# yeyupiaoling/VoiceprintRecognition-PaddlePaddle

Hardware: NVIDIA H100
Metric: utterances/sec ECAPA-TDNN Fbank80 3s embed extract (higher is better)
Workload: dtype bf16x3 (split-bf16 operands, fp32 accumulate; fp32-grade)

## Files before the change

voiceprintrecognition-paddlepaddle_b200/csrc/gemm_epilogue.cuh:

```cuda
#pragma once
#include "common.h"
#include "ptx.cuh"

namespace ppv {

constexpr int GEMM_MMA_THREADS = 256;
constexpr int GEMM_THREADS = 128 + GEMM_MMA_THREADS;

__device__ __forceinline__ float epilogue_math1(const Epilogue& ep, int N, int col, int64_t grp, int64_t sgrp, float x) {
    if (ep.bias) x += __ldg(ep.bias + col);
    if (ep.rowgrp_bias) x += __ldg(ep.rowgrp_bias + grp * N + col);
    if (ep.seg_scale) x *= __ldg(ep.seg_scale + sgrp * N + col);
    if (ep.relu) {
        x = fmaxf(x, 0.f);
        if (ep.relu_max > 0.f) x = fminf(x, ep.relu_max);
    }
    if (ep.silu_) x = x / (1.f + expf(-x));
    if (ep.bn_scale) x = fmaf(x, __ldg(ep.bn_scale + col), __ldg(ep.bn_shift + col));
    if (ep.tanh_) x = tanhf(x);
    if (ep.sigmoid_) x = 1.f / (1.f + expf(-x));
    return x;
}

struct EpiRow {
    bool valid = false;
    int64_t out_row = 0, mirror_a = -1, mirror_b = -1, grp = 0, sgrp = 0;
    int64_t zero_row = -1;
};
__device__ __forceinline__ EpiRow epilogue_row(const Epilogue& ep, int64_t row, int64_t out_row_shift) {
    EpiRow r;
    r.valid = row >= 0;
    const int64_t row_in = row;
    if (row < 0) row = 0;
    r.out_row = row + out_row_shift;
    if (ep.img_Wp > 0) {
        const int64_t img = int64_t(ep.img_Hp) * ep.img_Wp;
        r.grp = row / img;
        const int rem = int(row - r.grp * img);
        const int h = rem / ep.img_Wp - 1, w = rem % ep.img_Wp - 1;
        r.valid = r.valid && h >= 0 && h < ep.img_H && w >= 0 && w < ep.img_W;
        const int sw = ep.img_stride_w ? ep.img_stride_w : ep.img_stride;
        r.valid = r.valid && (h % ep.img_stride) == 0 && (w % sw) == 0;
        r.out_row = (r.grp * ep.out_Hp + h / ep.img_stride + 1) * ep.out_Wp + w / sw + 1;
    } else if (ep.Tp > 0) {
        r.grp = row / ep.Tp;
        const int t = int(row - r.grp * ep.Tp) - ep.P;
        r.valid = r.valid && t >= 0 && t < ep.T;
        if (ep.seg_scale && r.valid) r.sgrp = r.grp * ep.nseg + t / ep.seg_len;
        if (ep.halo && r.valid) {
            if (t >= 1 && t <= ep.P) r.mirror_a = row - 2 * t;
            const int u = ep.T - 1 - t;
            if (u >= 1 && u <= ep.P) r.mirror_b = row + 2 * u;
        }
    }
    const bool same_grid = ep.img_Wp == 0 || (ep.img_stride == 1 && ep.img_stride_w <= 1 && ep.out_Hp == ep.img_Hp && ep.out_Wp == ep.img_Wp);
    if (!r.valid && row_in >= 0 && ep.zero_invalid && ep.out_mode == OUT_PLANES && !ep.halo && same_grid) r.zero_row = row_in + out_row_shift;
    return r;
}

__device__ __forceinline__ void epilogue_pair(const Epilogue& ep, int N, int col, const EpiRow& r, float a, float b) {
    if (col >= N) return;
    if (!r.valid) {
        if (r.zero_row >= 0) {
            __nv_bfloat16* ph = static_cast<__nv_bfloat16*>(ep.out) + r.zero_row * ep.out_ld + ep.out_col0 + col;
            *reinterpret_cast<uint32_t*>(ph) = 0u;
            *reinterpret_cast<uint32_t*>(ph + ep.out_plane_stride) = 0u;
        }
        return;
    }
    const bool two = col + 1 < N;
    a = epilogue_math1(ep, N, col, r.grp, r.sgrp, a);
    if (two) b = epilogue_math1(ep, N, col + 1, r.grp, r.sgrp, b);
    if (ep.out_mode == OUT_F32) {
        float* dst = static_cast<float*>(ep.out) + r.out_row * ep.out_ld + ep.out_col0 + col;
        if (two && ep.f32_vec_ok) {
            *reinterpret_cast<float2*>(dst) = make_float2(a, b);
        } else {
            dst[0] = a;
            if (two) dst[1] = b;
        }
        return;
    }
    uint32_t h, l;
    split_pack_bf16x2(a, b, h, l);
    __nv_bfloat16* obase = static_cast<__nv_bfloat16*>(ep.out) + ep.out_col0 + col;
    auto store_row = [&](int64_t row) {
        uint32_t* ph = reinterpret_cast<uint32_t*>(obase + row * ep.out_ld);
        ph[0] = h;
        *reinterpret_cast<uint32_t*>(reinterpret_cast<__nv_bfloat16*>(ph) + ep.out_plane_stride) = l;
    };
    store_row(r.out_row);
    if (r.mirror_a >= 0) store_row(r.mirror_a);
    if (r.mirror_b >= 0) store_row(r.mirror_b);
}

template <int BN, typename RowOf>
__device__ __forceinline__ void epilogue_frag(const Epilogue& ep, int N, int n0, float (&acc)[BN / 2], RowOf&& row_of, int t,
                                              int64_t out_row_shift = 0) {
    if (ep.debug_nostore) return;
    const int w = t >> 5, l = t & 31;
    const int r0 = 16 * w + (l >> 2);
    const EpiRow ra = epilogue_row(ep, row_of(r0), out_row_shift);
    const EpiRow rb = epilogue_row(ep, row_of(r0 + 8), out_row_shift);
    constexpr int EPI_GROUPS = BN / 8 < 4 ? BN / 8 : 4;
#pragma unroll 1
    for (int c = 0; c < BN / 8; c += EPI_GROUPS) {
#pragma unroll
        for (int i = 0; i < EPI_GROUPS; ++i) {
            const int col = n0 + 8 * (c + i) + 2 * (l & 3);
            epilogue_pair(ep, N, col, ra, acc[4 * i + 0], acc[4 * i + 1]);
            epilogue_pair(ep, N, col, rb, acc[4 * i + 2], acc[4 * i + 3]);
        }
#pragma unroll
        for (int j = 0; j + 4 * EPI_GROUPS < BN / 2; ++j) acc[j] = acc[j + 4 * EPI_GROUPS];
    }
}

template <int BN, typename RowOf>
__device__ __forceinline__ void epilogue_frag_lean(const Epilogue& ep, int N, int n0, float (&acc)[BN / 2], RowOf&& row_of, int t) {
    static_assert(BN % 32 == 0, "lean epilogue: whole 32-column trips");
    const int w = t >> 5, l = t & 31, q = l & 3;
    const int r0 = 16 * w + (l >> 2);
    const EpiRow ra = epilogue_row(ep, row_of(r0), 0);
    const EpiRow rb = epilogue_row(ep, row_of(r0 + 8), 0);
    const int cq = n0 + 8 * q;
    __nv_bfloat16* const obase = static_cast<__nv_bfloat16*>(ep.out) + ep.out_col0 + cq;
    __nv_bfloat16* const pa = obase + ra.out_row * ep.out_ld;
    __nv_bfloat16* const pb = obase + rb.out_row * ep.out_ld;
    const int64_t lo_off = ep.out_plane_stride;
    const float* const ga = ep.rowgrp_bias ? ep.rowgrp_bias + ra.grp * N + cq : nullptr;
    const float* const gb = ep.rowgrp_bias ? ep.rowgrp_bias + rb.grp * N + cq : nullptr;
    const bool q2 = (q & 2) != 0, q1 = (q & 1) != 0;
#pragma unroll 1
    for (int c = 0; c < BN / 8; c += 4) {
        float a[8], b[8];
#pragma unroll
        for (int i = 0; i < 4; ++i) a[2 * i] = acc[4 * i], a[2 * i + 1] = acc[4 * i + 1], b[2 * i] = acc[4 * i + 2], b[2 * i + 1] = acc[4 * i + 3];
#pragma unroll
        for (int j = 0; j + 16 < BN / 2; ++j) acc[j] = acc[j + 16];
#pragma unroll
        for (int e = 0; e < 4; ++e) {
            const float sa = q2 ? a[e] : a[e + 4], sb = q2 ? b[e] : b[e + 4];
            const float ra_ = __shfl_xor_sync(0xffffffffu, sa, 2), rb_ = __shfl_xor_sync(0xffffffffu, sb, 2);
            if (q2) a[e] = ra_, b[e] = rb_;
            else a[e + 4] = ra_, b[e + 4] = rb_;
        }
#pragma unroll
        for (int e = 0; e < 8; e += 4) {
#pragma unroll
            for (int f = 0; f < 2; ++f) {
                const float sa = q1 ? a[e + f] : a[e + 2 + f], sb = q1 ? b[e + f] : b[e + 2 + f];
                const float ra_ = __shfl_xor_sync(0xffffffffu, sa, 1), rb_ = __shfl_xor_sync(0xffffffffu, sb, 1);
                if (q1) a[e + f] = ra_, b[e + f] = rb_;
                else a[e + 2 + f] = ra_, b[e + 2 + f] = rb_;
            }
        }
        const int j0 = 8 * c;
        if (n0 + j0 >= N) continue;
#pragma unroll
        for (int k = 0; k < 8; ++k) {
            const int col = cq + j0 + k;
            if (ep.bias) {
                const float bb = __ldg(ep.bias + col);
                a[k] += bb, b[k] += bb;
            }
            if (ga) a[k] += __ldg(ga + j0 + k), b[k] += __ldg(gb + j0 + k);
            if (ep.relu) a[k] = fmaxf(a[k], 0.f), b[k] = fmaxf(b[k], 0.f);
            if (ep.bn_scale) {
                const float sc = __ldg(ep.bn_scale + col), sh = __ldg(ep.bn_shift + col);
                a[k] = fmaf(a[k], sc, sh), b[k] = fmaf(b[k], sc, sh);
            }
            if (ep.tanh_) a[k] = tanhf(a[k]), b[k] = tanhf(b[k]);
        }
        uint4 ha, la, hb, lb;
        split_pack_bf16x2(a[0], a[1], ha.x, la.x), split_pack_bf16x2(a[2], a[3], ha.y, la.y);
        split_pack_bf16x2(a[4], a[5], ha.z, la.z), split_pack_bf16x2(a[6], a[7], ha.w, la.w);
        split_pack_bf16x2(b[0], b[1], hb.x, lb.x), split_pack_bf16x2(b[2], b[3], hb.y, lb.y);
        split_pack_bf16x2(b[4], b[5], hb.z, lb.z), split_pack_bf16x2(b[6], b[7], hb.w, lb.w);
        if (ra.valid) {
            *reinterpret_cast<uint4*>(pa + j0) = ha;
            *reinterpret_cast<uint4*>(pa + j0 + lo_off) = la;
        }
        if (rb.valid) {
            *reinterpret_cast<uint4*>(pb + j0) = hb;
            *reinterpret_cast<uint4*>(pb + j0 + lo_off) = lb;
        }
    }
}

template <int BN, typename RowOf>
__device__ __forceinline__ void gemm_epilogue(const Epilogue& ep, int N, int n0, float (&acc)[BN / 2], RowOf&& row_of, int t,
                                              int64_t out_row_shift) {
    if (ep.lean) epilogue_frag_lean<BN>(ep, N, n0, acc, row_of, t);
    else epilogue_frag<BN>(ep, N, n0, acc, row_of, t, out_row_shift);
}

}
```

voiceprintrecognition-paddlepaddle_b200/csrc/res2chain.cu:

```cuda
#include <stdio.h>
#include <stdlib.h>
#include <string.h>

#include "common.h"
#include "gemm_epilogue.cuh"
#include "ptx.cuh"

namespace ppv {

constexpr int RC_PAD = 4;
constexpr int RC_BOX_ROWS = 200;
constexpr int RC_ROWS = 2 * RC_BOX_ROWS;
constexpr int RC_A_PLANE = RC_ROWS * 128;
constexpr int RC_W_TILE = 64 * 128;
constexpr int RC_MAX_TILES = 3;
constexpr int RC_MAX_TP = RC_MAX_TILES * GEMM_BM;
constexpr int RC_S_PLANE = GEMM_BM * 128;
constexpr int RC_MMA_THREADS = 128 * RC_MAX_TILES;
constexpr int RC_THREADS = 128 + RC_MMA_THREADS;

template <int NSPLIT>
struct RCCfg {
    static constexpr int NP = (NSPLIT == 3) ? 2 : 1;
    static constexpr int A_BYTES = NP * RC_A_PLANE;
    static constexpr int W_SLOT = 3 * NP * RC_W_TILE;
    static constexpr int S_BYTES = NP * RC_S_PLANE;
    static constexpr int SMEM_BYTES = 1024 + A_BYTES + W_SLOT + 2 * S_BYTES + 256;
};

__device__ __forceinline__ void rp_st_global(bool pred, uint32_t* p, uint32_t v) {
    asm volatile("{\n\t.reg .pred p;\n\tsetp.ne.b32 p, %2, 0;\n\t@p st.global.u32 [%0], %1;\n\t}" ::"l"(p), "r"(v), "r"(uint32_t(pred)) : "memory");
}
__device__ __forceinline__ void rp_st_shared(bool pred, uint32_t a, uint32_t v) {
    asm volatile("{\n\t.reg .pred p;\n\tsetp.ne.b32 p, %2, 0;\n\t@p st.shared.u32 [%0], %1;\n\t}" ::"r"(a), "r"(v), "r"(uint32_t(pred)) : "memory");
}

__device__ __forceinline__ uint32_t rc_ld_shared(uint32_t a) {
    uint32_t v;
    asm volatile("ld.shared.u32 %0, [%1];" : "=r"(v) : "r"(a) : "memory");
    return v;
}

#define RC_STAMP(role, conv, ev)                                                                   \
    do {                                                                                          \
        if (cp.trace && blockIdx.x == 0 && b == 0) cp.trace[((role) * 8 + (conv)) * 8 + (ev)] = clock64(); \
    } while (0)

template <int NSPLIT>
__global__ void __launch_bounds__(RC_THREADS, 1) res2chain_kernel(const __grid_constant__ Res2ChainParams cp) {
    using Cfg = RCCfg<NSPLIT>;
    constexpr int NP = Cfg::NP, BN = 64;
    extern __shared__ uint8_t smem_raw[];
    const uint32_t smem_base = (smem_u32(smem_raw) + 1023u) & ~1023u;
    uint8_t* smem_gen = smem_raw + (smem_base - smem_u32(smem_raw));
    const uint32_t a_base = smem_base;
    const uint32_t w_base = a_base + Cfg::A_BYTES;
    const uint32_t s_base = w_base + Cfg::W_SLOT;
    const uint32_t bar_base = s_base + 2 * Cfg::S_BYTES;
    const uint32_t x_full = bar_base, x_free = bar_base + 24, w_full = bar_base + 32, w_empty = bar_base + 40;
    auto s_full = [&](int i) { return bar_base + 48u + 8u * i; };
    auto s_empty = [&](int i) { return bar_base + 64u + 8u * i; };
    auto y_ready = [&](int i) { return bar_base + 80u + 8u * i; };

    const int warp = threadIdx.x >> 5, lane = threadIdx.x & 31;
    if (warp == 0 && lane == 0) {
        prefetch_tmap(&cp.mapX);
        prefetch_tmap(&cp.mapXt);
        prefetch_tmap(&cp.mapY);
        prefetch_tmap(&cp.mapYtail);
        for (int j = 0; j < cp.nconv; ++j) prefetch_tmap(&cp.mapW[j]);
    }
    if (warp == 1 && lane == 0) {
        mbar_init(x_full, 1);
        mbar_init(x_free, 1);
        mbar_init(w_full, 1);
        mbar_init(w_empty, 1);
        for (int i = 0; i < 2; ++i) {
            mbar_init(s_full(i), 1);
            mbar_init(s_empty(i), 1);
            mbar_init(y_ready(i), 128);
        }
        fence_mbar_init();
    }
    __syncthreads();
    griddep_launch_dependents();
    const int nconv = cp.nconv, ntiles = cp.ntiles;

    if (warp == 0) {
        if (lane == 0) {
            griddep_wait();
            int g = 0, u = 0;
            uint32_t sn = 0;
            for (int b = blockIdx.x; b < cp.B; b += gridDim.x, ++u) {
                if (u > 0) mbar_wait(x_free, uint32_t(u - 1) & 1u);
                mbar_arrive_expect_tx(x_full, NP * 2 * RC_BOX_ROWS * 128);
                for (int pl = 0; pl < NP; ++pl)
                    for (int h = 0; h < 2; ++h)
                        tma_load_3d(a_base + pl * RC_A_PLANE + h * RC_BOX_ROWS * 128, &cp.mapX, x_full, cp.width ,
                                    b * cp.Tp - RC_PAD + h * RC_BOX_ROWS, pl);
                for (int j = 0; j < nconv; ++j, ++g) {
                    if (g > 0) mbar_wait(w_empty, uint32_t(g - 1) & 1u);
                    RC_STAMP(0, j, 0);
                    mbar_arrive_expect_tx(w_full, 3 * NP * RC_W_TILE);
                    for (int tap = 0; tap < 3; ++tap)
                        for (int pl = 0; pl < NP; ++pl) tma_load_3d(w_base + (tap * NP + pl) * RC_W_TILE, &cp.mapW[j], w_full, tap * 64, 0, pl);
                    for (int t = 0; t < ntiles; ++t, ++sn) {
                        const int i = sn & 1;
                        if (sn >= 2) mbar_wait(s_empty(i), ((sn >> 1) - 1) & 1u);
                        if (j + 1 < nconv) {
                            mbar_arrive_expect_tx(s_full(i), NP * RC_S_PLANE);
                            for (int pl = 0; pl < NP; ++pl)
                                tma_load_3d(s_base + i * Cfg::S_BYTES + pl * RC_S_PLANE, &cp.mapXt, s_full(i), (j + 2) * cp.width,
                                            b * cp.Tp + t * GEMM_BM, pl);
                        } else {
                            mbar_arrive(s_full(i));
                        }
                    }
                }
            }
        }
    } else if (warp == 3) {
        if (lane == 0) {
            uint32_t sn = 0;
            for (int b = blockIdx.x; b < cp.B; b += gridDim.x) {
                for (int j = 0; j < nconv; ++j) {
                    for (int t = 0; t < ntiles; ++t, ++sn) {
                        const int i = sn & 1;
                        mbar_wait(y_ready(i), (sn >> 1) & 1u);
                        const CUtensorMap* my = (t == ntiles - 1) ? &cp.mapYtail : &cp.mapY;
                        for (int pl = 0; pl < NP; ++pl)
                            tma_store_3d(my, s_base + i * Cfg::S_BYTES + pl * RC_S_PLANE, (j + 1) * cp.width, b * cp.Tp + t * GEMM_BM, pl);
                        bulk_commit_group();
                        bulk_wait_read0();
                        mbar_arrive(s_empty(i));
                    }
                }
            }
            bulk_wait_all();
        }
    } else if (warp >= 4) {
        const int tw = (warp - 4) >> 2, tid = threadIdx.x & 127, w = tid >> 5, l = tid & 31;
        const int e = threadIdx.x - 128;
        const bool has_tile = tw < ntiles;
        griddep_wait();
        uint8_t* const a_gen = smem_gen;
        float acc0[BN / 2], acc1[BN / 2];
#pragma unroll
        for (int i = 0; i < BN / 2; ++i) acc0[i] = acc1[i] = 0.f;
        uint32_t g = 0, ucount = 0;
        for (int b = blockIdx.x; b < cp.B; b += gridDim.x, ++ucount) {
            {
                mbar_wait(x_full, ucount & 1u);
                if (e < 2 * cp.P * 8 * NP) {
                    const int pl = e / (2 * cp.P * 8), r = (e / 8) % (2 * cp.P), c = e % 8;
                    const int k = (r % cp.P) + 1;
                    const int dst = (r < cp.P ? cp.P - k : cp.P + cp.T - 1 + k) + RC_PAD, src = (r < cp.P ? cp.P + k : cp.P + cp.T - 1 - k) + RC_PAD;
                    const uint4 val = *reinterpret_cast<const uint4*>(a_gen + pl * RC_A_PLANE + src * 128 + ((c ^ (src & 7)) << 4));
                    *reinterpret_cast<uint4*>(a_gen + pl * RC_A_PLANE + dst * 128 + ((c ^ (dst & 7)) << 4)) = val;
                }
                fence_proxy_async_smem();
                named_bar_sync(1, RC_MMA_THREADS);
            }
            for (int j = 0; j < nconv; ++j, ++g) {
                mbar_wait(w_full, g & 1u);
                if (tid == 0 && tw == 0) RC_STAMP(1, j, 1);
                if (has_tile) {
                    wgmma_fence_acc(acc0);
                    wgmma_fence_acc(acc1);
                    wgmma_fence();
                    auto issue = [&](float (&acc)[BN / 2], int mb) {
#pragma unroll
                        for (int tap = 0; tap < 3; ++tap) {
                            const uint32_t roff = uint32_t(tw * GEMM_BM + mb * 64 + RC_PAD + (tap - 1) * cp.dil);
                            const uint64_t a_hi = make_sw128_kmajor_desc(a_base + roff * 128u);
                            const uint64_t b_hi = make_sw128_kmajor_desc(w_base + (tap * NP) * RC_W_TILE);
#pragma unroll
                            for (int k = 0; k < 4; ++k) wgmma_bf16<BN>(acc, a_hi + 2 * k, b_hi + 2 * k, (tap > 0 || k > 0) ? 1u : 0u);
                            if (NSPLIT == 3) {
                                const uint64_t a_lo = make_sw128_kmajor_desc(a_base + RC_A_PLANE + roff * 128u);
                                const uint64_t b_lo = make_sw128_kmajor_desc(w_base + (tap * NP + 1) * RC_W_TILE);
#pragma unroll
                                for (int k = 0; k < 4; ++k) wgmma_bf16<BN>(acc, a_lo + 2 * k, b_hi + 2 * k, 1u);
#pragma unroll
                                for (int k = 0; k < 4; ++k) wgmma_bf16<BN>(acc, a_hi + 2 * k, b_lo + 2 * k, 1u);
                            }
                        }
                    };
                    issue(acc0, 0);
                    issue(acc1, 1);
                    wgmma_commit();
                    wgmma_wait<0>();
                    wgmma_fence_acc(acc0);
                    wgmma_fence_acc(acc1);
                }
                named_bar_sync(1, RC_MMA_THREADS);
                if (e == 0) {
                    RC_STAMP(1, j, 2);
                    mbar_arrive(w_empty);
                    if (j == nconv - 1) mbar_arrive(x_free);
                }
                const float* bias = cp.bias[j];
                const float* bsc = cp.bn_scale[j];
                const float* bsh = cp.bn_shift[j];
                const bool has_next = j + 1 < nconv;
                const uint32_t sn = g * uint32_t(ntiles) + uint32_t(tw);
                const int i = sn & 1;
                auto epilogue = [&](const float (&acc)[BN / 2], int mb) {
#pragma unroll 1
                    for (int h = 0; h < 2; ++h) {
                        const int rloc = mb * 64 + 16 * w + (l >> 2) + 8 * h;
                        const int p = tw * GEMM_BM + rloc;
                        const int tt = p - cp.P, uu = cp.T - 1 - tt;
                        const bool next = has_next && tt >= 0 && tt < cp.T;
                        const int m0 = p + RC_PAD;
                        const int m1 = (tt >= 1 && tt <= cp.P) ? cp.P - tt + RC_PAD : -1;
                        const int m2 = (uu >= 1 && uu <= cp.P) ? cp.P + cp.T - 1 + uu + RC_PAD : -1;
                        const uint32_t srow = s_base + i * Cfg::S_BYTES + rloc * 128 + 4 * (l & 3);
#pragma unroll
                        for (int q = 0; q < BN / 8; ++q) {
                            const int col = 8 * q + 2 * (l & 3);
                            const uint32_t so = srow + ((q ^ (rloc & 7)) << 4);
                            const float2 b2 = __ldg(reinterpret_cast<const float2*>(bias + col));
                            const float2 s2 = __ldg(reinterpret_cast<const float2*>(bsc + col));
                            const float2 h2 = __ldg(reinterpret_cast<const float2*>(bsh + col));
                            const float a0 = h ? acc[4 * q + 2] : acc[4 * q], a1 = h ? acc[4 * q + 3] : acc[4 * q + 1];
                            const float x0 = fmaf(fmaxf(a0 + b2.x, 0.f), s2.x, h2.x);
                            const float x1 = fmaf(fmaxf(a1 + b2.y, 0.f), s2.y, h2.y);
                            uint32_t nh = 0, nl = 0;
                            if (has_next) {
                                nh = rc_ld_shared(so);
                                if (NP == 2) nl = rc_ld_shared(so + RC_S_PLANE);
                            }
                            uint32_t yh, yl;
                            split_pack_bf16x2(x0, x1, yh, yl);
                            rp_st_shared(true, so, yh);
                            if (NP == 2) rp_st_shared(true, so + RC_S_PLANE, yl);
                            const float2 hf = unpack_bf16x2(nh), lf = unpack_bf16x2(nl);
                            uint32_t oh, ol;
                            split_pack_bf16x2(x0 + (hf.x + lf.x), x1 + (hf.y + lf.y), oh, ol);
                            auto put = [&](bool pred, int row) {
                                const uint32_t d = a_base + row * 128 + ((q ^ (row & 7)) << 4) + 4 * (l & 3);
                                rp_st_shared(pred, d, oh);
                                if (NP == 2) rp_st_shared(pred, d + RC_A_PLANE, ol);
                            };
                            put(next, m0);
                            put(next && m1 >= 0, m1);
                            put(next && m2 >= 0, m2);
                        }
                    }
                };
#pragma unroll 1
                for (int round = 0; round < 2; ++round) {
                    if (has_tile && (tw == 2) == (round == 1)) {
                        mbar_wait(s_full(i), (sn >> 1) & 1u);
                        epilogue(acc0, 0);
                        epilogue(acc1, 1);
                        fence_proxy_async_smem();
                        mbar_arrive(y_ready(i));
                    }
                    if (ntiles > 2 && round == 0) named_bar_sync(2, RC_MMA_THREADS);
                }
                if (tid == 0 && tw == 0) RC_STAMP(2, j, 5);
                if (has_next) {
                    fence_proxy_async_smem();
                    named_bar_sync(1, RC_MMA_THREADS);
                }
            }
        }
    }
}

constexpr int RP_BLOCKS = 5;
constexpr int RP_MAX_TP = RP_BLOCKS * 64;
constexpr int RP_BOX_ROWS = 168;
constexpr int RP_A_PLANE = 2 * RP_BOX_ROWS * 128;
constexpr int RP_THREADS = 128 * RP_BLOCKS;
constexpr int RP_VEC_FLOATS = 3 * RES2CHAIN_MAX * 64;

template <int NSPLIT>
struct RPCfg {
    static constexpr int NP = (NSPLIT == 3) ? 2 : 1;
    static constexpr int U_BYTES = NP * RP_A_PLANE;
    static constexpr int W_SLOT = 3 * NP * RC_W_TILE;
    static constexpr int SMEM_BYTES = 1024 + 2 * U_BYTES + W_SLOT + RP_VEC_FLOATS * 4 + 64;
};
static_assert(RPCfg<3>::SMEM_BYTES <= 232448, "paired res2chain exceeds the H100 shared-memory opt-in");

#define RP_STAMP(role, conv, ev)                                                                                \
    do {                                                                                                        \
        if (trace_on) cp.trace[((role) * 8 + (conv)) * 8 + (ev)] = clock64();                                   \
    } while (0)

__device__ __forceinline__ int rp_opaque(int v) {
    asm volatile("mov.b32 %0, %0;" : "+r"(v));
    return v;
}

template <int NSPLIT>
__global__ void __launch_bounds__(RP_THREADS, 1) res2chain_pair_kernel(const __grid_constant__ Res2ChainParams cp) {
    using Cfg = RPCfg<NSPLIT>;
    constexpr int NP = Cfg::NP, BN = 64;
    extern __shared__ uint8_t smem_raw[];
    const uint32_t smem_base = (smem_u32(smem_raw) + 1023u) & ~1023u;
    uint8_t* const a_gen = smem_raw + (smem_base - smem_u32(smem_raw));
    const uint32_t w_base = smem_base + 2 * Cfg::U_BYTES;
    float* const vec = reinterpret_cast<float*>(a_gen + 2 * Cfg::U_BYTES + Cfg::W_SLOT);
    const uint32_t bar_base = w_base + Cfg::W_SLOT + RP_VEC_FLOATS * 4;
    const uint32_t x_full = bar_base, w_full = bar_base + 8;

    const int tid = threadIdx.x, wg = tid >> 7, wq = (tid >> 5) & 3, l = tid & 31;
    const int nconv = cp.nconv, T = cp.T, P = cp.P, Tp = cp.Tp;
    if (tid == 0) {
        prefetch_tmap(&cp.mapX);
        for (int j = 0; j < nconv; ++j) prefetch_tmap(&cp.mapW[j]);
        mbar_init(x_full, 1);
        mbar_init(w_full, 1);
        fence_mbar_init();
    }
    __syncthreads();
    griddep_launch_dependents();
    griddep_wait();
    for (int i = tid; i < 3 * 64 * nconv; i += RP_THREADS) {
        const int j = i / 192, k = (i / 64) % 3, c = i % 64;
        vec[i] = (k == 0 ? cp.bias[j] : k == 1 ? cp.bn_scale[j] : cp.bn_shift[j])[c];
    }

    auto load_w = [&](int j) {
        mbar_arrive_expect_tx(w_full, 3 * NP * RC_W_TILE);
        for (int tap = 0; tap < 3; ++tap)
            for (int pl = 0; pl < NP; ++pl) tma_load_3d(w_base + (tap * NP + pl) * RC_W_TILE, &cp.mapW[j], w_full, tap * 64, 0, pl);
    };
    auto prefetch_chunk = [&](int b0, int c) {
        for (int u = 0; u < 2 && b0 + u < cp.B; ++u)
            for (int pl = 0; pl < NP; ++pl)
                for (int h = 0; h < 2; ++h) tma_prefetch_l2_3d(&cp.mapX, c * cp.width, (b0 + u) * Tp - RC_PAD + h * RP_BOX_ROWS, pl);
    };
    auto issue = [&](float (&acc)[BN / 2], int u) {
        wgmma_fence_acc(acc);
        wgmma_fence();
#pragma unroll
        for (int tap = 0; tap < 3; ++tap) {
            const uint32_t a_row = smem_base + rp_opaque(u * Cfg::U_BYTES) + uint32_t(wg * 64 + RC_PAD + (tap - 1) * cp.dil) * 128u;
            const uint64_t a_hi = make_sw128_kmajor_desc(a_row);
            const uint64_t b_hi = make_sw128_kmajor_desc(w_base + (tap * NP) * RC_W_TILE);
#pragma unroll
            for (int k = 0; k < 4; ++k) wgmma_bf16<BN>(acc, a_hi + 2 * k, b_hi + 2 * k, (tap > 0 || k > 0) ? 1u : 0u);
            if (NSPLIT == 3) {
                const uint64_t a_lo = make_sw128_kmajor_desc(a_row + RP_A_PLANE);
                const uint64_t b_lo = make_sw128_kmajor_desc(w_base + (tap * NP + 1) * RC_W_TILE);
#pragma unroll
                for (int k = 0; k < 4; ++k) wgmma_bf16<BN>(acc, a_lo + 2 * k, b_hi + 2 * k, 1u);
#pragma unroll
                for (int k = 0; k < 4; ++k) wgmma_bf16<BN>(acc, a_hi + 2 * k, b_lo + 2 * k, 1u);
            }
        }
        wgmma_commit();
    };
    auto epilogue = [&](const float (&acc)[BN / 2], int u, int b, int j) {
        b = rp_opaque(b);
        const bool present = b < cp.B, has_next = j + 1 < nconv;
        const float* const vb = vec + j * 192 + 2 * (l & 3);
        const uint32_t tile = smem_base + u * Cfg::U_BYTES;
#pragma unroll 1
        for (int part = 0; part < 8; ++part) {
            const int h = part >> 2, qh = 2 * (part & 3);
            const int r = wg * 64 + 16 * wq + (l >> 2) + 8 * h;
            const int tt = r - P, uu = T - 1 - tt;
            const bool store = present && r < Tp;
            const bool next = has_next && store && tt >= 0 && tt < T;
            const int m0 = r + RC_PAD;
            const int m1 = (tt >= 1 && tt <= P) ? P - tt + RC_PAD : -1;
            const int m2 = (uu >= 1 && uu <= P) ? P + T - 1 + uu + RC_PAD : -1;
            const int64_t grow = int64_t(b) * Tp + r;
            const uint32_t* const xh = reinterpret_cast<const uint32_t*>(cp.x.hi() + grow * cp.x.ld + (j + 2) * cp.width + 2 * (l & 3)) + 4 * qh;
            uint32_t* const yh = reinterpret_cast<uint32_t*>(cp.y.hi() + grow * cp.y.ld + (j + 1) * cp.width + 2 * (l & 3)) + 4 * qh;
            const int64_t xlo = cp.x.plane_stride / 2, ylo = cp.y.plane_stride / 2;
            uint32_t nh[2], nl[2];
#pragma unroll
            for (int i = 0; i < 2; ++i) {
                nh[i] = next ? __ldg(xh + 4 * i) : 0u;
                nl[i] = (next && NP == 2) ? __ldg(xh + 4 * i + xlo) : 0u;
            }
#pragma unroll
            for (int i = 0; i < 2; ++i) {
                const int q = qh + i;
                const float2 b2 = *reinterpret_cast<const float2*>(vb + 8 * q);
                const float2 s2 = *reinterpret_cast<const float2*>(vb + 64 + 8 * q);
                const float2 h2 = *reinterpret_cast<const float2*>(vb + 128 + 8 * q);
                float a0 = acc[4 * i], a1 = acc[4 * i + 1];
#pragma unroll
                for (int k = 0; k < 8; ++k)
                    if (part == k) a0 = acc[4 * (2 * (k & 3) + i) + 2 * (k >> 2)], a1 = acc[4 * (2 * (k & 3) + i) + 2 * (k >> 2) + 1];
                const float x0 = fmaf(fmaxf(a0 + b2.x, 0.f), s2.x, h2.x);
                const float x1 = fmaf(fmaxf(a1 + b2.y, 0.f), s2.y, h2.y);
                uint32_t vh, vl;
                split_pack_bf16x2(x0, x1, vh, vl);
                rp_st_global(store, yh + 4 * i, vh);
                if (NP == 2) rp_st_global(store, yh + 4 * i + ylo, vl);
                const float2 hf = unpack_bf16x2(nh[i]), lf = unpack_bf16x2(nl[i]);
                uint32_t oh, ol;
                split_pack_bf16x2(x0 + (hf.x + lf.x), x1 + (hf.y + lf.y), oh, ol);
                auto put = [&](bool pred, int row) {
                    const uint32_t d = tile + row * 128 + ((q ^ (row & 7)) << 4) + 4 * (l & 3);
                    rp_st_shared(pred, d, oh);
                    if (NP == 2) rp_st_shared(pred, d + RP_A_PLANE, ol);
                };
                put(next, m0);
                put(next && m1 >= 0, m1);
                put(next && m2 >= 0, m2);
            }
        }
    };

    float accA[BN / 2], accB[BN / 2];
#pragma unroll
    for (int i = 0; i < BN / 2; ++i) accA[i] = accB[i] = 0.f;
    const int npairs = (cp.B + 1) / 2;
    uint32_t g = 0, it = 0;
    for (int pi = blockIdx.x; pi < npairs; pi += gridDim.x, ++it) {
        const int b0 = 2 * pi;
        const bool trace_on = cp.trace && blockIdx.x == 0 && it == 0 && tid == 0;
        if (tid == 0) {
            mbar_arrive_expect_tx(x_full, 2 * NP * RP_A_PLANE);
            for (int u = 0; u < 2; ++u)
                for (int pl = 0; pl < NP; ++pl)
                    for (int h = 0; h < 2; ++h)
                        tma_load_3d(smem_base + u * Cfg::U_BYTES + pl * RP_A_PLANE + h * RP_BOX_ROWS * 128, &cp.mapX, x_full,
                                    cp.width , (b0 + u) * Tp - RC_PAD + h * RP_BOX_ROWS, pl);
            RP_STAMP(2, 0, 0);
            load_w(0);
            for (int c = 2; c <= 3 && c <= nconv; ++c) prefetch_chunk(b0, c);
        }
        {
            mbar_wait(x_full, it & 1u);
            const int per_u = 2 * P * 8 * NP;
            if (tid < 2 * per_u) {
                const int u = tid / per_u, e = tid % per_u;
                const int pl = e / (2 * P * 8), r = (e / 8) % (2 * P), c = e % 8;
                const int k = (r % P) + 1;
                const int dst = (r < P ? P - k : P + T - 1 + k) + RC_PAD, src = (r < P ? P + k : P + T - 1 - k) + RC_PAD;
                uint8_t* const base = a_gen + u * Cfg::U_BYTES + pl * RP_A_PLANE;
                *reinterpret_cast<uint4*>(base + dst * 128 + ((c ^ (dst & 7)) << 4)) =
                    *reinterpret_cast<const uint4*>(base + src * 128 + ((c ^ (src & 7)) << 4));
            }
            fence_proxy_async_smem();
            __syncthreads();
        }
        for (int j = 0; j < nconv; ++j, ++g) {
            mbar_wait(w_full, g & 1u);
            RP_STAMP(2, j, 1);
            if (tid == 0 && j + 3 <= nconv) prefetch_chunk(b0, j + 3);
            issue(accA, 0);
            wgmma_wait<1>();
            RP_STAMP(0, j, 0);
            if (j > 0) {
                RP_STAMP(1, j - 1, 2);
                epilogue(accB, 1, b0 + 1, j - 1);
                RP_STAMP(1, j - 1, 3);
                fence_proxy_async_smem();
            }
            __syncthreads();
            issue(accB, 1);
            RP_STAMP(1, j, 0);
            wgmma_wait<1>();
            wgmma_fence_acc(accA);
            __syncthreads();
            RP_STAMP(0, j, 1);
            RP_STAMP(0, j, 2);
            epilogue(accA, 0, b0, j);
            RP_STAMP(0, j, 3);
            fence_proxy_async_smem();
            wgmma_wait<0>();
            wgmma_fence_acc(accB);
            __syncthreads();
            RP_STAMP(1, j, 1);
            if (tid == 0 && j + 1 < nconv) {
                RP_STAMP(2, j + 1, 0);
                load_w(j + 1);
            }
        }
        RP_STAMP(1, nconv - 1, 2);
        epilogue(accB, 1, b0 + 1, nconv - 1);
        RP_STAMP(1, nconv - 1, 3);
        __syncthreads();
    }
}

int res2chain_build(Res2ChainParams* cp, const Planes& x, const Planes& y, const Planes* W, const float* const* bias, const float* const* bn_scale,
                    const float* const* bn_shift, int nconv, int B, int T, int P, int Tp, int dil, bool paired) {
    PPV_REQUIRE(nconv >= 1 && nconv <= RES2CHAIN_MAX, "res2chain: 1..7 convs");
    PPV_REQUIRE(P == RC_PAD && Tp == T + 2 * P && Tp <= RC_MAX_TP, "res2chain: padded utterance must fit 384 rows with P == 4");
    PPV_REQUIRE(!paired || Tp <= RP_MAX_TP, "res2chain: the paired kernel needs a padded utterance of at most 320 rows");
    PPV_REQUIRE(dil >= 1 && dil <= RC_PAD, "res2chain: dilation must be in [1,4]");
    PPV_REQUIRE(x.ld >= (nconv + 1) * 64 && y.ld >= (nconv + 1) * 64, "res2chain: buffers narrower than the chunks");
    memset(static_cast<void*>(cp), 0, sizeof(*cp));
    int rc = encode_planes_map_ex(&cp->mapX, x, 64, paired ? RP_BOX_ROWS : RC_BOX_ROWS, 128);
    if (rc) return rc;
    const int ntiles = (Tp + GEMM_BM - 1) / GEMM_BM;
    if (!paired) {
        rc = encode_planes_map_ex(&cp->mapXt, x, 64, GEMM_BM, 128);
        if (rc) return rc;
        rc = encode_planes_map_ex(&cp->mapY, y, 64, GEMM_BM, 128);
        if (rc) return rc;
        rc = encode_planes_map_ex(&cp->mapYtail, y, 64, Tp - (ntiles - 1) * GEMM_BM, 128);
        if (rc) return rc;
    }
    for (int j = 0; j < nconv; ++j) {
        PPV_REQUIRE(W[j].ld >= 192 && W[j].rows >= 64, "res2chain: weight layout mismatch");
        rc = encode_planes_map(&cp->mapW[j], W[j], 64);
        if (rc) return rc;
        cp->bias[j] = bias[j];
        cp->bn_scale[j] = bn_scale[j];
        cp->bn_shift[j] = bn_shift[j];
    }
    cp->x = x;
    cp->y = y;
    cp->nconv = nconv;
    cp->width = 64;
    cp->B = B;
    cp->T = T;
    cp->P = P;
    cp->Tp = Tp;
    cp->dil = dil;
    cp->ntiles = ntiles;
    cp->paired = paired ? 1 : 0;
    if (getenv("PPV_RES2_TRACE")) {
        static unsigned long long* buf = nullptr;
        if (!buf) {
            cudaMalloc(reinterpret_cast<void**>(&buf), 3 * 8 * 8 * sizeof(unsigned long long));
            cudaMemset(buf, 0, 3 * 8 * 8 * sizeof(unsigned long long));
        }
        cp->trace = buf;
    }
    return PPV_OK;
}

template <int NSPLIT>
static int launch_rc(const Res2ChainParams& cp, int num_sms, cudaStream_t st) {
    using Cfg = RCCfg<NSPLIT>;
    PPV_ONCE_PER_DEVICE(PPV_CUDA_OK(cudaFuncSetAttribute(res2chain_kernel<NSPLIT>, cudaFuncAttributeMaxDynamicSharedMemorySize, Cfg::SMEM_BYTES)));
    const int grid = std::min(cp.B, num_sms);
    PPV_PDL_OK(launch_pdl(res2chain_kernel<NSPLIT>, dim3(grid), dim3(RC_THREADS), Cfg::SMEM_BYTES, st, cp), "res2chain_kernel");
    return PPV_OK;
}

template <int NSPLIT>
static int launch_rp(const Res2ChainParams& cp, int num_sms, cudaStream_t st) {
    using Cfg = RPCfg<NSPLIT>;
    PPV_ONCE_PER_DEVICE(PPV_CUDA_OK(cudaFuncSetAttribute(res2chain_pair_kernel<NSPLIT>, cudaFuncAttributeMaxDynamicSharedMemorySize, Cfg::SMEM_BYTES)));
    const int grid = std::min((cp.B + 1) / 2, num_sms);
    PPV_PDL_OK(launch_pdl(res2chain_pair_kernel<NSPLIT>, dim3(grid), dim3(RP_THREADS), Cfg::SMEM_BYTES, st, cp), "res2chain_pair_kernel");
    return PPV_OK;
}

int res2chain_launch(const Res2ChainParams& cp, int precision, int num_sms, cudaStream_t st) {
    if (cp.paired) return precision == PPV_PREC_BF16X3 ? launch_rp<3>(cp, num_sms, st) : launch_rp<1>(cp, num_sms, st);
    return precision == PPV_PREC_BF16X3 ? launch_rc<3>(cp, num_sms, st) : launch_rc<1>(cp, num_sms, st);
}
void res2chain_trace_dump(const Res2ChainParams& cp) {
    if (!cp.trace) return;
    unsigned long long h[3 * 8 * 8];
    cudaDeviceSynchronize();
    cudaMemcpy(h, cp.trace, sizeof(h), cudaMemcpyDeviceToHost);
    unsigned long long t0 = ~0ull;
    for (unsigned long long v : h)
        if (v && v < t0) t0 = v;
    static const char* const single_roles[3] = {"tma", "mma", "epi"};
    static const char* const pair_roles[3] = {"utt A", "utt B", "weights"};
    const char* const* roles = cp.paired ? pair_roles : single_roles;
    for (int r = 0; r < 3; ++r)
        for (int j = 0; j < 7; ++j) {
            printf("res2chain trace %s conv %d:", roles[r], j);
            for (int e = 0; e < 8; ++e) printf(" %8lld", h[(r * 8 + j) * 8 + e] ? (long long)(h[(r * 8 + j) * 8 + e] - t0) : -1ll);
            printf("\n");
        }
}
bool res2chain_fits(int T, int P) { return P == RC_PAD && T + 2 * P <= RC_MAX_TP; }
bool res2chain_pair_fits(int T, int P) { return P == RC_PAD && T + 2 * P <= RP_MAX_TP; }

}
```

Baseline: 34950.

## Stage next res2 chunk via TMA and vectorize paired-kernel epilogue stores

The paired res2chain epilogue now quad-transposes accumulators so each lane owns 8 contiguous columns. This allows 16-byte vector global stores of the y output and 16-byte shared loads and stores. The next chunk's input x is no longer read per element with __ldg. Instead it is prefetched by TMA into the shared A tile under new per-utterance mbarriers, so the residual add reads it from shared memory. This trades extra barrier and parity bookkeeping, and a new 16-byte alignment requirement on y, for fewer scattered global accesses in the epilogue.

```diff
diff --git a/voiceprintrecognition-paddlepaddle_b200/csrc/gemm_epilogue.cuh b/voiceprintrecognition-paddlepaddle_b200/csrc/gemm_epilogue.cuh
--- a/voiceprintrecognition-paddlepaddle_b200/csrc/gemm_epilogue.cuh
+++ b/voiceprintrecognition-paddlepaddle_b200/csrc/gemm_epilogue.cuh
@@ -116,6 +116,27 @@
     }
 }
 
+__device__ __forceinline__ void quad_transpose_pairs(float (&a)[8], float (&b)[8], int q) {
+    const bool q2 = (q & 2) != 0, q1 = (q & 1) != 0;
+#pragma unroll
+    for (int e = 0; e < 4; ++e) {
+        const float sa = q2 ? a[e] : a[e + 4], sb = q2 ? b[e] : b[e + 4];
+        const float ra_ = __shfl_xor_sync(0xffffffffu, sa, 2), rb_ = __shfl_xor_sync(0xffffffffu, sb, 2);
+        if (q2) a[e] = ra_, b[e] = rb_;
+        else a[e + 4] = ra_, b[e + 4] = rb_;
+    }
+#pragma unroll
+    for (int e = 0; e < 8; e += 4) {
+#pragma unroll
+        for (int f = 0; f < 2; ++f) {
+            const float sa = q1 ? a[e + f] : a[e + 2 + f], sb = q1 ? b[e + f] : b[e + 2 + f];
+            const float ra_ = __shfl_xor_sync(0xffffffffu, sa, 1), rb_ = __shfl_xor_sync(0xffffffffu, sb, 1);
+            if (q1) a[e + f] = ra_, b[e + f] = rb_;
+            else a[e + 2 + f] = ra_, b[e + 2 + f] = rb_;
+        }
+    }
+}
+
 template <int BN, typename RowOf>
 __device__ __forceinline__ void epilogue_frag_lean(const Epilogue& ep, int N, int n0, float (&acc)[BN / 2], RowOf&& row_of, int t) {
     static_assert(BN % 32 == 0, "lean epilogue: whole 32-column trips");
@@ -130,7 +151,6 @@
     const int64_t lo_off = ep.out_plane_stride;
     const float* const ga = ep.rowgrp_bias ? ep.rowgrp_bias + ra.grp * N + cq : nullptr;
     const float* const gb = ep.rowgrp_bias ? ep.rowgrp_bias + rb.grp * N + cq : nullptr;
-    const bool q2 = (q & 2) != 0, q1 = (q & 1) != 0;
 #pragma unroll 1
     for (int c = 0; c < BN / 8; c += 4) {
         float a[8], b[8];
@@ -138,23 +158,7 @@
         for (int i = 0; i < 4; ++i) a[2 * i] = acc[4 * i], a[2 * i + 1] = acc[4 * i + 1], b[2 * i] = acc[4 * i + 2], b[2 * i + 1] = acc[4 * i + 3];
 #pragma unroll
         for (int j = 0; j + 16 < BN / 2; ++j) acc[j] = acc[j + 16];
-#pragma unroll
-        for (int e = 0; e < 4; ++e) {
-            const float sa = q2 ? a[e] : a[e + 4], sb = q2 ? b[e] : b[e + 4];
-            const float ra_ = __shfl_xor_sync(0xffffffffu, sa, 2), rb_ = __shfl_xor_sync(0xffffffffu, sb, 2);
-            if (q2) a[e] = ra_, b[e] = rb_;
-            else a[e + 4] = ra_, b[e + 4] = rb_;
-        }
-#pragma unroll
-        for (int e = 0; e < 8; e += 4) {
-#pragma unroll
-            for (int f = 0; f < 2; ++f) {
-                const float sa = q1 ? a[e + f] : a[e + 2 + f], sb = q1 ? b[e + f] : b[e + 2 + f];
-                const float ra_ = __shfl_xor_sync(0xffffffffu, sa, 1), rb_ = __shfl_xor_sync(0xffffffffu, sb, 1);
-                if (q1) a[e + f] = ra_, b[e + f] = rb_;
-                else a[e + 2 + f] = ra_, b[e + 2 + f] = rb_;
-            }
-        }
+        quad_transpose_pairs(a, b, q);
         const int j0 = 8 * c;
         if (n0 + j0 >= N) continue;
 #pragma unroll
diff --git a/voiceprintrecognition-paddlepaddle_b200/csrc/res2chain.cu b/voiceprintrecognition-paddlepaddle_b200/csrc/res2chain.cu
--- a/voiceprintrecognition-paddlepaddle_b200/csrc/res2chain.cu
+++ b/voiceprintrecognition-paddlepaddle_b200/csrc/res2chain.cu
@@ -28,11 +28,23 @@
     static constexpr int SMEM_BYTES = 1024 + A_BYTES + W_SLOT + 2 * S_BYTES + 256;
 };
 
-__device__ __forceinline__ void rp_st_global(bool pred, uint32_t* p, uint32_t v) {
-    asm volatile("{\n\t.reg .pred p;\n\tsetp.ne.b32 p, %2, 0;\n\t@p st.global.u32 [%0], %1;\n\t}" ::"l"(p), "r"(v), "r"(uint32_t(pred)) : "memory");
-}
 __device__ __forceinline__ void rp_st_shared(bool pred, uint32_t a, uint32_t v) {
     asm volatile("{\n\t.reg .pred p;\n\tsetp.ne.b32 p, %2, 0;\n\t@p st.shared.u32 [%0], %1;\n\t}" ::"r"(a), "r"(v), "r"(uint32_t(pred)) : "memory");
+}
+__device__ __forceinline__ void rp_st_global_v4(bool pred, const void* p, uint4 v) {
+    asm volatile("{\n\t.reg .pred p;\n\tsetp.ne.b32 p, %5, 0;\n\t@p st.global.v4.u32 [%0], {%1, %2, %3, %4};\n\t}" ::"l"(p), "r"(v.x), "r"(v.y),
+                 "r"(v.z), "r"(v.w), "r"(uint32_t(pred))
+                 : "memory");
+}
+__device__ __forceinline__ void rp_st_shared_v4(bool pred, uint32_t a, uint4 v) {
+    asm volatile("{\n\t.reg .pred p;\n\tsetp.ne.b32 p, %5, 0;\n\t@p st.shared.v4.u32 [%0], {%1, %2, %3, %4};\n\t}" ::"r"(a), "r"(v.x), "r"(v.y),
+                 "r"(v.z), "r"(v.w), "r"(uint32_t(pred))
+                 : "memory");
+}
+__device__ __forceinline__ uint4 rp_ld_shared_v4(uint32_t a) {
+    uint4 v;
+    asm volatile("ld.shared.v4.u32 {%0, %1, %2, %3}, [%4];" : "=r"(v.x), "=r"(v.y), "=r"(v.z), "=r"(v.w) : "r"(a) : "memory");
+    return v;
 }
 
 __device__ __forceinline__ uint32_t rc_ld_shared(uint32_t a) {
@@ -307,6 +319,7 @@
     float* const vec = reinterpret_cast<float*>(a_gen + 2 * Cfg::U_BYTES + Cfg::W_SLOT);
     const uint32_t bar_base = w_base + Cfg::W_SLOT + RP_VEC_FLOATS * 4;
     const uint32_t x_full = bar_base, w_full = bar_base + 8;
+    auto x_next = [&](int u) { return bar_base + 16u + 8u * u; };
 
     const int tid = threadIdx.x, wg = tid >> 7, wq = (tid >> 5) & 3, l = tid & 31;
     const int nconv = cp.nconv, T = cp.T, P = cp.P, Tp = cp.Tp;
@@ -315,6 +328,8 @@
         for (int j = 0; j < nconv; ++j) prefetch_tmap(&cp.mapW[j]);
         mbar_init(x_full, 1);
         mbar_init(w_full, 1);
+        mbar_init(x_next(0), 1);
+        mbar_init(x_next(1), 1);
         fence_mbar_init();
     }
     __syncthreads();
@@ -329,6 +344,12 @@
         mbar_arrive_expect_tx(w_full, 3 * NP * RC_W_TILE);
         for (int tap = 0; tap < 3; ++tap)
             for (int pl = 0; pl < NP; ++pl) tma_load_3d(w_base + (tap * NP + pl) * RC_W_TILE, &cp.mapW[j], w_full, tap * 64, 0, pl);
+    };
+    auto load_x = [&](uint32_t bar, int u, int b, int c) {
+        for (int pl = 0; pl < NP; ++pl)
+            for (int h = 0; h < 2; ++h)
+                tma_load_3d(smem_base + u * Cfg::U_BYTES + pl * RP_A_PLANE + h * RP_BOX_ROWS * 128, &cp.mapX, bar, c * cp.width,
+                            b * Tp - RC_PAD + h * RP_BOX_ROWS, pl);
     };
     auto prefetch_chunk = [&](int b0, int c) {
         for (int u = 0; u < 2 && b0 + u < cp.B; ++u)
@@ -356,54 +377,75 @@
         }
         wgmma_commit();
     };
-    auto epilogue = [&](const float (&acc)[BN / 2], int u, int b, int j) {
+    bool trace_on = false;
+    auto epilogue = [&](float (&acc)[BN / 2], int u, int b, int j, uint32_t xpar) {
         b = rp_opaque(b);
         const bool present = b < cp.B, has_next = j + 1 < nconv;
-        const float* const vb = vec + j * 192 + 2 * (l & 3);
+        j = rp_opaque(j);
+        const int q = l & 3, r0 = wg * 64 + 16 * wq + (l >> 2);
+#pragma unroll
+        for (int c = 0; c < 2; ++c) {
+            float a[8], bb[8];
+#pragma unroll
+            for (int i = 0; i < 4; ++i)
+                a[2 * i] = acc[16 * c + 4 * i], a[2 * i + 1] = acc[16 * c + 4 * i + 1], bb[2 * i] = acc[16 * c + 4 * i + 2],
+                bb[2 * i + 1] = acc[16 * c + 4 * i + 3];
+            quad_transpose_pairs(a, bb, q);
+            const float* const vb = vec + j * 192 + 32 * c + 8 * q;
+#pragma unroll
+            for (int k4 = 0; k4 < 8; k4 += 4) {
+                const float4 b4 = *reinterpret_cast<const float4*>(vb + k4);
+                const float4 s4 = *reinterpret_cast<const float4*>(vb + 64 + k4);
+                const float4 h4 = *reinterpret_cast<const float4*>(vb + 128 + k4);
+                const float bv[4] = {b4.x, b4.y, b4.z, b4.w}, sv[4] = {s4.x, s4.y, s4.z, s4.w}, hv[4] = {h4.x, h4.y, h4.z, h4.w};
+#pragma unroll
+                for (int k = 0; k < 4; ++k) {
+                    acc[16 * c + k4 + k] = fmaf(fmaxf(a[k4 + k] + bv[k], 0.f), sv[k], hv[k]);
+                    acc[16 * c + 8 + k4 + k] = fmaf(fmaxf(bb[k4 + k] + bv[k], 0.f), sv[k], hv[k]);
+                }
+            }
+#pragma unroll
+            for (int h = 0; h < 2; ++h) {
+                const float* const v = acc + 16 * c + 8 * h;
+                const int r = r0 + 8 * h;
+                const __nv_bfloat16* const yp = cp.y.hi() + (int64_t(b) * Tp + r) * cp.y.ld + (j + 1) * cp.width + 32 * c + 8 * q;
+                uint4 vh, vl;
+                split_pack_bf16x2(v[0], v[1], vh.x, vl.x), split_pack_bf16x2(v[2], v[3], vh.y, vl.y);
+                split_pack_bf16x2(v[4], v[5], vh.z, vl.z), split_pack_bf16x2(v[6], v[7], vh.w, vl.w);
+                rp_st_global_v4(present && r < Tp, yp, vh);
+                if (NP == 2) rp_st_global_v4(present && r < Tp, yp + cp.y.plane_stride, vl);
+            }
+        }
+        RP_STAMP(u, j, 5);
+        if (!(present && has_next)) return;
+        mbar_wait(x_next(u), xpar);
+        RP_STAMP(u, j, 6);
         const uint32_t tile = smem_base + u * Cfg::U_BYTES;
-#pragma unroll 1
-        for (int part = 0; part < 8; ++part) {
-            const int h = part >> 2, qh = 2 * (part & 3);
-            const int r = wg * 64 + 16 * wq + (l >> 2) + 8 * h;
-            const int tt = r - P, uu = T - 1 - tt;
-            const bool store = present && r < Tp;
-            const bool next = has_next && store && tt >= 0 && tt < T;
-            const int m0 = r + RC_PAD;
-            const int m1 = (tt >= 1 && tt <= P) ? P - tt + RC_PAD : -1;
-            const int m2 = (uu >= 1 && uu <= P) ? P + T - 1 + uu + RC_PAD : -1;
-            const int64_t grow = int64_t(b) * Tp + r;
-            const uint32_t* const xh = reinterpret_cast<const uint32_t*>(cp.x.hi() + grow * cp.x.ld + (j + 2) * cp.width + 2 * (l & 3)) + 4 * qh;
-            uint32_t* const yh = reinterpret_cast<uint32_t*>(cp.y.hi() + grow * cp.y.ld + (j + 1) * cp.width + 2 * (l & 3)) + 4 * qh;
-            const int64_t xlo = cp.x.plane_stride / 2, ylo = cp.y.plane_stride / 2;
-            uint32_t nh[2], nl[2];
-#pragma unroll
-            for (int i = 0; i < 2; ++i) {
-                nh[i] = next ? __ldg(xh + 4 * i) : 0u;
-                nl[i] = (next && NP == 2) ? __ldg(xh + 4 * i + xlo) : 0u;
-            }
-#pragma unroll
-            for (int i = 0; i < 2; ++i) {
-                const int q = qh + i;
-                const float2 b2 = *reinterpret_cast<const float2*>(vb + 8 * q);
-                const float2 s2 = *reinterpret_cast<const float2*>(vb + 64 + 8 * q);
-                const float2 h2 = *reinterpret_cast<const float2*>(vb + 128 + 8 * q);
-                float a0 = acc[4 * i], a1 = acc[4 * i + 1];
-#pragma unroll
-                for (int k = 0; k < 8; ++k)
-                    if (part == k) a0 = acc[4 * (2 * (k & 3) + i) + 2 * (k >> 2)], a1 = acc[4 * (2 * (k & 3) + i) + 2 * (k >> 2) + 1];
-                const float x0 = fmaf(fmaxf(a0 + b2.x, 0.f), s2.x, h2.x);
-                const float x1 = fmaf(fmaxf(a1 + b2.y, 0.f), s2.y, h2.y);
-                uint32_t vh, vl;
-                split_pack_bf16x2(x0, x1, vh, vl);
-                rp_st_global(store, yh + 4 * i, vh);
-                if (NP == 2) rp_st_global(store, yh + 4 * i + ylo, vl);
-                const float2 hf = unpack_bf16x2(nh[i]), lf = unpack_bf16x2(nl[i]);
-                uint32_t oh, ol;
-                split_pack_bf16x2(x0 + (hf.x + lf.x), x1 + (hf.y + lf.y), oh, ol);
+        const int r1 = rp_opaque(r0);
+#pragma unroll
+        for (int c = 0; c < 2; ++c) {
+#pragma unroll
+            for (int h = 0; h < 2; ++h) {
+                const int r = r1 + 8 * h, tt = r - P, uu = T - 1 - tt;
+                const bool next = tt >= 0 && tt < T;
+                const int m0 = r + RC_PAD;
+                const int m1 = (tt >= 1 && tt <= P) ? P - tt + RC_PAD : -1;
+                const int m2 = (uu >= 1 && uu <= P) ? P + T - 1 + uu + RC_PAD : -1;
+                const int k16 = 4 * c + q;
+                const uint32_t s0 = tile + m0 * 128 + ((k16 ^ (m0 & 7)) << 4);
+                const uint4 xh = rp_ld_shared_v4(s0);
+                const uint4 xl = NP == 2 ? rp_ld_shared_v4(s0 + RP_A_PLANE) : make_uint4(0u, 0u, 0u, 0u);
+                const float* const v = acc + 16 * c + 8 * h;
+                uint4 oh, ol;
+                auto add = [&](uint32_t nh, uint32_t nl, int k, uint32_t& ph, uint32_t& pl) {
+                    const float2 hf = unpack_bf16x2(nh), lf = unpack_bf16x2(nl);
+                    split_pack_bf16x2(v[k] + (hf.x + lf.x), v[k + 1] + (hf.y + lf.y), ph, pl);
+                };
+                add(xh.x, xl.x, 0, oh.x, ol.x), add(xh.y, xl.y, 2, oh.y, ol.y), add(xh.z, xl.z, 4, oh.z, ol.z), add(xh.w, xl.w, 6, oh.w, ol.w);
                 auto put = [&](bool pred, int row) {
-                    const uint32_t d = tile + row * 128 + ((q ^ (row & 7)) << 4) + 4 * (l & 3);
-                    rp_st_shared(pred, d, oh);
-                    if (NP == 2) rp_st_shared(pred, d + RP_A_PLANE, ol);
+                    const uint32_t d = tile + row * 128 + ((k16 ^ (row & 7)) << 4);
+                    rp_st_shared_v4(pred, d, oh);
+                    if (NP == 2) rp_st_shared_v4(pred, d + RP_A_PLANE, ol);
                 };
                 put(next, m0);
                 put(next && m1 >= 0, m1);
@@ -419,14 +461,10 @@
     uint32_t g = 0, it = 0;
     for (int pi = blockIdx.x; pi < npairs; pi += gridDim.x, ++it) {
         const int b0 = 2 * pi;
-        const bool trace_on = cp.trace && blockIdx.x == 0 && it == 0 && tid == 0;
+        trace_on = cp.trace && blockIdx.x == 0 && it == 0 && tid == 0;
         if (tid == 0) {
             mbar_arrive_expect_tx(x_full, 2 * NP * RP_A_PLANE);
-            for (int u = 0; u < 2; ++u)
-                for (int pl = 0; pl < NP; ++pl)
-                    for (int h = 0; h < 2; ++h)
-                        tma_load_3d(smem_base + u * Cfg::U_BYTES + pl * RP_A_PLANE + h * RP_BOX_ROWS * 128, &cp.mapX, x_full,
-                                    cp.width , (b0 + u) * Tp - RC_PAD + h * RP_BOX_ROWS, pl);
+            for (int u = 0; u < 2; ++u) load_x(x_full, u, b0 + u, 1);
             RP_STAMP(2, 0, 0);
             load_w(0);
             for (int c = 2; c <= 3 && c <= nconv; ++c) prefetch_chunk(b0, c);
@@ -455,7 +493,7 @@
             RP_STAMP(0, j, 0);
             if (j > 0) {
                 RP_STAMP(1, j - 1, 2);
-                epilogue(accB, 1, b0 + 1, j - 1);
+                epilogue(accB, 1, b0 + 1, j - 1, (g - 1 - it) & 1u);
                 RP_STAMP(1, j - 1, 3);
                 fence_proxy_async_smem();
             }
@@ -466,8 +504,13 @@
             wgmma_fence_acc(accA);
             __syncthreads();
             RP_STAMP(0, j, 1);
+            if (tid == 0 && j + 1 < nconv) {
+                mbar_arrive_expect_tx(x_next(0), NP * RP_A_PLANE);
+                load_x(x_next(0), 0, b0, j + 2);
+                RP_STAMP(0, j, 4);
+            }
             RP_STAMP(0, j, 2);
-            epilogue(accA, 0, b0, j);
+            epilogue(accA, 0, b0, j, (g - it) & 1u);
             RP_STAMP(0, j, 3);
             fence_proxy_async_smem();
             wgmma_wait<0>();
@@ -477,10 +520,15 @@
             if (tid == 0 && j + 1 < nconv) {
                 RP_STAMP(2, j + 1, 0);
                 load_w(j + 1);
+                if (b0 + 1 < cp.B) {
+                    mbar_arrive_expect_tx(x_next(1), NP * RP_A_PLANE);
+                    load_x(x_next(1), 1, b0 + 1, j + 2);
+                    RP_STAMP(1, j, 4);
+                }
             }
         }
         RP_STAMP(1, nconv - 1, 2);
-        epilogue(accB, 1, b0 + 1, nconv - 1);
+        epilogue(accB, 1, b0 + 1, nconv - 1, 0u);
         RP_STAMP(1, nconv - 1, 3);
         __syncthreads();
     }
@@ -497,7 +545,9 @@
     int rc = encode_planes_map_ex(&cp->mapX, x, 64, paired ? RP_BOX_ROWS : RC_BOX_ROWS, 128);
     if (rc) return rc;
     const int ntiles = (Tp + GEMM_BM - 1) / GEMM_BM;
-    if (!paired) {
+    if (paired) {
+        PPV_REQUIRE(!(reinterpret_cast<uintptr_t>(y.base) & 15) && y.ld % 8 == 0 && y.plane_stride % 8 == 0, "res2chain: y planes not 16-byte aligned");
+    } else {
         rc = encode_planes_map_ex(&cp->mapXt, x, 64, GEMM_BM, 128);
         if (rc) return rc;
         rc = encode_planes_map_ex(&cp->mapY, y, 64, GEMM_BM, 128);
```

Result: faster. 36780, median of 6 (+5.2%).
